# OSU-Bee-Lab/buzzdetect

Measured on AMD Instinct MI355X. Metric: yamnet_windows_per_s, higher is better.
Workload: dtype f32 (split-f16x3 MFMA products, f32 accumulate)

## Files before the change

### buzzdetect_amd/csrc/bd_internal.h

```cpp
#pragma once

#include <hip/hip_runtime.h>
#include <stdint.h>

#include <vector>

#include "../../include/buzzdetect_hip.h"

namespace bd {

constexpr int kMelNonZero = 461;

constexpr int kMelStart[BD_MEL_BANDS] = {
    5, 5, 6, 7, 9, 10, 11, 12, 13, 14, 16, 17, 18, 20, 21, 23, 25, 26, 28, 30, 32, 34, 36, 38, 40, 42, 44, 47, 49, 52, 54, 57,
    60, 63, 66, 69, 72, 76, 79, 83, 87, 90, 95, 99, 103, 108, 112, 117, 122, 127, 133, 138, 144, 150, 156, 162, 169, 176, 183,
    190, 198, 206, 214, 223};
constexpr int kMelLen[BD_MEL_BANDS] = {
    1, 2, 3, 3, 2, 2, 2, 2, 3, 3, 2, 3, 3, 3, 4, 3, 3, 4, 4, 4, 4, 4, 4, 4, 4, 5, 5, 5, 5, 5, 6, 6,
    6, 6, 6, 7, 7, 7, 8, 7, 8, 9, 8, 9, 9, 9, 10, 10, 11, 11, 11, 12, 12, 12, 13, 14, 14, 14, 15, 16, 16, 17, 17, 17};
constexpr int mel_offset(int band) {
    int o = 0;
    for (int m = 0; m < band; ++m) o += kMelLen[m];
    return o;
}
// ... 96 lines not shown
                                   unsigned* range_flag = nullptr);
void launch_scale_copy(const float* src, float* dst, int64_t n, float factor, hipStream_t stream);
bool launch_pointwise_next_dw_f32(const float* in, float* out, int windows, const SepLayer& L, const SepLayer& Ln,
                                  hipStream_t stream);
bool launch_l4_reg_f32(const float* in, float* out, int windows, const SepLayer& L4, const SepLayer& L5, hipStream_t stream);
bool launch_separable_chip(const float* in, float* out, int windows, const SepLayer* L, int nl, hipStream_t stream,
                           const SepLayer* next = nullptr, bool planes = false);
bool tail_supported(const SepLayer& L13, const SepLayer& L14);
bool launch_tail_pw13_dw14(const void* in, void* out, int windows, const SepLayer& L13, const SepLayer& L14, hipStream_t stream);
bool launch_tail_pw14_pool(const void* in, float* pooled, int windows, const SepLayer& L14, hipStream_t stream);
bool tail_f32_supported(const SepLayer& L13, const SepLayer& L14);
bool launch_tail_f32(const float* in, float* mid, float* pooled, int windows, const SepLayer& L13, const SepLayer& L14, hipStream_t stream,
                     int which);
bool launch_separable_chip_f32(const float* in, float* out, int windows, const SepLayer* L, int nl, hipStream_t stream,
                               const SepLayer* next, bool dw0_done);
bool launch_separable_mid_f32(const float* in, float* out, int windows, const SepLayer& L5, const SepLayer& L6, const SepLayer& L7,
                              hipStream_t stream);
bool launch_separable_mid(const float* in, float* out, int windows, const SepLayer& L5, const SepLayer& L6, const SepLayer& L7,
                          hipStream_t stream);
int launch_separable_run_next_dw(const float* a, float* b, int windows, const SepLayer* L, int max_layers, hipStream_t stream,
                                 bool planes = false);
bool launch_separable_fused_next_dw(const float* in, float* out, int windows, const SepLayer& L, const SepLayer& next,
                                    hipStream_t stream);
void launch_stem_reg(const float* logmel, int patch_step, const WindowMap& map, int w0, int windows, const float* c1_w,
                     const float* c1_b, const SepLayer& L2, const SepLayer& L3, float* out, hipStream_t stream);
void launch_stem_reg_f32(const float* logmel, int patch_step, const WindowMap& map, int w0, int windows, const float* c1_w,
                         const float* c1_b, const SepLayer& L2, const SepLayer& L3, float* out, hipStream_t stream);
void launch_stem4(const float* logmel, int patch_step, const WindowMap& map, int w0, int windows, const float* c1_w,
                  const float* c1_b,
                  const SepLayer& L2, const SepLayer& L3, float* out, hipStream_t stream);
void launch_pool_head(const float* act, int windows, const float* head_wt, const float* head_b,
                      int n_classes, float* emb, float* logits, hipStream_t stream);
void launch_head(const float* pooled, int windows, const float* head_wt, const float* head_b, int n_classes,
                 float* logits, hipStream_t stream);

}
```

### buzzdetect_amd/csrc/cnn.hip

```cpp
#include "bd_internal.h"
#include <mutex>
#include <type_traits>

namespace bd {

namespace {

typedef float f32x16 __attribute__((ext_vector_type(16)));

constexpr float kF16Max = 65504.0f;
__device__ __forceinline__ float range_of(float m, float4 v) {
    return fmaxf(fmaxf(m, fabsf(v.x)), fmaxf(fmaxf(fabsf(v.y), fabsf(v.z)), fabsf(v.w)));
}
typedef float v4f_range __attribute__((ext_vector_type(4)));
__device__ __forceinline__ float range_of(float m, v4f_range v) {
    return fmaxf(fmaxf(m, fabsf(v.x)), fmaxf(fmaxf(fabsf(v.y), fabsf(v.z)), fabsf(v.w)));
}
__device__ __forceinline__ void range_report(float m, unsigned* __restrict__ flag) {
    if (flag && !(m <= kF16Max)) *flag = 1u;
}

constexpr int kMaxDevices = 64;
template <typename Kernel>
void allow_dynamic_lds(Kernel kernel, int bytes, std::once_flag (&once)[kMaxDevices]) {
// ... 1207 lines not shown
    }
#undef BD_R_LOAD
#undef BD_R_SPLIT1
    range_report(rmax, range_flag);
}

template <int K16, bool PLAIN = false>
void launch_pw_res(const float* X, const SepLayer& L, float* out, int M, hipStream_t stream) {
    if constexpr (!PLAIN) {
        if (L.pw_mode == 2) return launch_pw_res<K16, true>(X, L, out, M, stream);
    }
    constexpr int lds = 2 * 2 * 32 * 32 * K16;
    static std::once_flag lds_once[kMaxDevices];
    allow_dynamic_lds(&pw_res_kernel<K16, PLAIN>, lds, lds_once);
    const int tiles_n = L.cout / 256;
    const int n_tiles = (M + 31) / 32;
    int streams = 256 / tiles_n;
    if (streams > n_tiles) streams = (n_tiles + 7) / 8 * 8;
    hipLaunchKernelGGL((pw_res_kernel<K16, PLAIN>), dim3((unsigned)(streams * tiles_n)), dim3(512), lds, stream, X,
                       static_cast<const _Float16*>(L.pw_fhi), static_cast<const _Float16*>(L.pw_flo), L.pw_u, L.pw_b, out, M,
                       L.cout, tiles_n, L.range_flag);
}

template <bool PLAIN>
__global__ __launch_bounds__(768) void l4_window_kernel(
    const float* __restrict__ X, const float* __restrict__ dw_w, const float* __restrict__ dw_b,
    const _Float16* __restrict__ Wfhi, const _Float16* __restrict__ Wflo, const float* __restrict__ pw_u,
    const float* __restrict__ pw_b,
    const float* __restrict__ ndw_w, const float* __restrict__ ndw_b, float* __restrict__ out, int windows,
    unsigned* __restrict__ range_flag) {
    constexpr int H = 24, W = 16, C = 128, K16 = 8, STEPS = H / 2;
    constexpr int COL_B = C * 4;
    constexpr int ROW_B = (W + 1) * COL_B;
    constexpr int RING0 = COL_B;
    constexpr int A0 = RING0 + 8 * ROW_B;
    constexpr int A_HALF = 32 * 2 * C, A_BUF = 2 * A_HALF;
    constexpr int T5 = A0 + 2 * A_BUF;
    constexpr int O5 = T5 + C * 12 * 4;
    constexpr int O5_ROW = (W / 2) * C * 4, O5_BUF = 2 * O5_ROW;
    constexpr size_t WIN_IN = (size_t)H * W * C, WIN_OUT = (size_t)STEPS * (W / 2) * C;
    static_assert(A0 % 512 == 0, "fragment addresses are formed by XOR");
    static_assert((2 * STEPS) % 8 == 0 && STEPS % 2 == 0, "ring slots and buffer parities carry over from window to window");
    extern __shared__ __attribute__((aligned(1024))) char smem_raw[];
    char* const smem = smem_raw;
    const int tid = threadIdx.x, lane = tid & 63;
    const int wave = __builtin_amdgcn_readfirstlane(tid >> 6);
    const int b = blockIdx.x, G = gridDim.x;
    if (b >= windows) return;
    const int NT = STEPS * ((windows - b + G - 1) / G);

    for (int i = tid; i < 9 * 32; i += 768) {
        const int z = i >> 5;
        *reinterpret_cast<v4f*>(smem + (z == 0 ? 0 : RING0 + (z - 1) * ROW_B + W * COL_B) + (i & 31) * 16) = v4f{0.f, 0.f, 0.f, 0.f};
    }
    for (int i = tid; i < 10 * C; i += 768) {
        const int t = i / C, c = i - t * C;
        reinterpret_cast<float*>(smem + T5)[c * 12 + t] = t < 9 ? ndw_w[t * C + c] : ndw_b[c];
    }
    float rmax = 0.0f;

    if (wave < 4) {
        const int frow = lane & 31, fh = lane >> 5;
        const int c4 = tid & 31, col_lo = tid >> 5;
        const float* const xt = X + (size_t)b * WIN_IN + (size_t)col_lo * C + c4 * 4;
        char* const ring_t = smem + RING0 + col_lo * COL_B + c4 * 16;
        v4f rs[2][4];
#define BD_L4_LOAD(DST, J)                                                                                \
    {                                                                                                     \
        const int i_ = (J) / STEPS, j_ = (J) - i_ * STEPS;                                                \
        const float* const src_ = xt + (size_t)i_ * G * WIN_IN + (size_t)j_ * (2 * W * C);                \
        _Pragma("unroll") for (int u = 0; u < 4; ++u)                                                     \
            DST[u] = *reinterpret_cast<const v4f*>(src_ + ((u >> 1) * W + 8 * (u & 1)) * C);              \
    }
#define BD_L4_STORE(SRC, J)                                                                               \
    _Pragma("unroll") for (int u = 0; u < 4; ++u)                                                         \
        *reinterpret_cast<v4f*>(ring_t + ((2 * (J) + (u >> 1)) & 7) * ROW_B + 8 * (u & 1) * COL_B) = SRC[u];
        BD_L4_LOAD(rs[0], 0)
        BD_L4_LOAD(rs[1], 1)
        f16x8 bh[K16], bl[K16];
#pragma unroll
        for (int q = 0; q < K16; ++q) {
            const size_t frag = ((size_t)(wave * K16 + q) * 64 + lane) * 8;
            bh[q] = *reinterpret_cast<const f16x8*>(Wfhi + frag);
            if constexpr (!PLAIN) bl[q] = *reinterpret_cast<const f16x8*>(Wflo + frag);
        }
        const int ncol = 32 * wave + frow;
        const float bcol = pw_b[ncol], ucol = pw_u[ncol];
        const float* const t5 = reinterpret_cast<const float*>(smem + T5) + ncol * 12;
        float acc5[4] = {0.0f, 0.0f, 0.0f, 0.0f};
        float* const o5 = reinterpret_cast<float*>(smem + O5) + (2 * fh) * C + ncol;
        int s5 = 0;
        BD_L4_STORE(rs[0], 0)
        BD_L4_STORE(rs[1], 1)
        BD_L4_LOAD(rs[0], 2)
        BD_L4_LOAD(rs[1], 3)
#pragma unroll
        for (int q = 0; q < K16; ++q) {
            bh[q] = pw_landed(bh[q]);
            if constexpr (!PLAIN) bl[q] = pw_landed(bl[q]);
        }
        const unsigned fr0 = pw_lds_addr(smem) + (unsigned)(A0 + frow * 2 * C + ((fh ^ (frow & 15)) << 4));
        __syncthreads();
        auto step = [&](auto pc, int k) {
            constexpr int p = decltype(pc)::value;
            f32x16 acc;
            if (k >= 1 && k <= NT) {
                const unsigned ab = fr0 + (unsigned)((p ^ 1) * A_BUF);
                using S = PwResSchedule<K16, 0, PLAIN ? 1 : 2>;
#pragma unroll
                for (int e = 0; e < 16; ++e) acc[e] = 0.0f;
                f16x8 fa[3][2];
#pragma unroll
                for (int q = 0; q < 2; ++q) {
                    fa[q][0] = pw_lds_frag<0>(ab ^ (q << 5));
                    if constexpr (!PLAIN) fa[q][1] = pw_lds_frag<A_HALF>(ab ^ (q << 5));
                }
                static_for_pw<0, K16>([&](auto qi) {
                    constexpr int q = decltype(qi)::value;
                    if constexpr (q + 2 < K16) {
                        fa[(q + 2) % 3][0] = pw_lds_frag<0>(ab ^ ((q + 2) << 5));
                        if constexpr (!PLAIN) fa[(q + 2) % 3][1] = pw_lds_frag<A_HALF>(ab ^ ((q + 2) << 5));
                    }
                    pw_lds_wait<S::pending(q)>();
                    const f16x8 ah = pw_landed(fa[q % 3][0]);
                    if constexpr (!PLAIN) {
                        const f16x8 al = pw_landed(fa[q % 3][1]);
                        acc = __builtin_amdgcn_mfma_f32_32x32x16_f16(al, bh[q], acc, 0, 0, 0);
                        acc = __builtin_amdgcn_mfma_f32_32x32x16_f16(ah, bl[q], acc, 0, 0, 0);
                    }
                    acc = __builtin_amdgcn_mfma_f32_32x32x16_f16(ah, bh[q], acc, 0, 0, 0);
                });
            }
            if (k + 2 < NT) { BD_L4_STORE(rs[p], k + 2) }
            if (k + 4 < NT) BD_L4_LOAD(rs[p], k + 4)
            if (k >= 1 && k <= NT) {
                float y[2][8], nb[2][2];
                const v4f t5a = *reinterpret_cast<const v4f*>(t5), t5b = *reinterpret_cast<const v4f*>(t5 + 4), t5c = *reinterpret_cast<const v4f*>(t5 + 8);
                const float w5[9] = {t5a.x, t5a.y, t5a.z, t5a.w, t5b.x, t5b.y, t5b.z, t5b.w, t5c.x};
                const float b5 = t5c.y;
#pragma unroll
                for (int e = 0; e < 16; ++e) y[e >> 3][e & 7] = fmaxf(fmaf(acc[e], ucol, bcol), 0.0f);
#pragma unroll
                for (int r = 0; r < 2; ++r) {
                    float va = y[r][0], wa = y[r][4], vb = y[r][4], wb = 0.0f;
                    asm("" : "+v"(va), "+v"(wa), "+v"(vb), "+v"(wb));
                    const auto s1 = __builtin_amdgcn_permlane32_swap(__builtin_bit_cast(unsigned, va), __builtin_bit_cast(unsigned, wa), false, false);
                    const auto s2 = __builtin_amdgcn_permlane32_swap(__builtin_bit_cast(unsigned, vb), __builtin_bit_cast(unsigned, wb), false, false);
                    nb[r][0] = __builtin_bit_cast(float, fh ? (unsigned)s1[0] : (unsigned)s1[1]);
                    nb[r][1] = fh ? 0.0f : __builtin_bit_cast(float, (unsigned)s2[1]);
                }
#define BD_L4_IN(R, T, KW) ((T) == 0 ? y[R][KW] : (T) == 1 ? ((KW) < 2 ? y[R][2 + (KW)] : nb[R][0]) : (T) == 2 ? y[R][4 + (KW)] : ((KW) < 2 ? y[R][6 + (KW)] : nb[R][1]))
                float* const orow = o5 + (p ^ 1) * (O5_BUF / 4);
                if (s5 > 0) {
#pragma unroll
                    for (int t = 0; t < 4; ++t) {
#pragma unroll
                        for (int kw = 0; kw < 3; ++kw) acc5[t] = fmaf(BD_L4_IN(0, t, kw), w5[6 + kw], acc5[t]);
// ... 1 lines not shown
                    }
                }
#pragma unroll
                for (int t = 0; t < 4; ++t) {
                    acc5[t] = b5;
#pragma unroll
                    for (int kh = 0; kh < 2; ++kh)
#pragma unroll
                        for (int kw = 0; kw < 3; ++kw) acc5[t] = fmaf(BD_L4_IN(kh, t, kw), w5[3 * kh + kw], acc5[t]);
                }
                if (s5 == STEPS - 1) {
#pragma unroll
                    for (int t = 0; t < 4; ++t) {
#pragma unroll
                        for (int kw = 0; kw < 3; ++kw) acc5[t] = fmaf(0.0f, w5[6 + kw], acc5[t]);
                        orow[((W / 2) + (t >> 1) * 4 + (t & 1)) * C] = fmaxf(acc5[t], 0.0f);
                    }
                    s5 = 0;
                } else {
                    ++s5;
                }
#undef BD_L4_IN
            }
            __syncthreads();
        };
        for (int k = 0; k < NT + 2; k += 2) {
            step(std::integral_constant<int, 0>{}, k);
            step(std::integral_constant<int, 1>{}, k + 1);
        }
#undef BD_L4_LOAD
#undef BD_L4_STORE
    } else {
        const int v = wave - 4, c4 = lane & 31;
        const int col = v < 4 ? 2 * (2 * v + (lane >> 5)) : 2 * (2 * (v - 4) + (lane >> 5)) + 1;
        v4f w4[9];
#pragma unroll
        for (int t = 0; t < 9; ++t) w4[t] = *reinterpret_cast<const v4f*>(dw_w + t * C + c4 * 4);
        const v4f b4 = *reinterpret_cast<const v4f*>(dw_b + c4 * 4);
        const char* const xin = smem + RING0 + (col - 1) * COL_B + c4 * 16;
        int a_st[2];
#pragma unroll
        for (int rr = 0; rr < 2; ++rr) {
            const int m = 16 * rr + col;
            a_st[rr] = A0 + m * 2 * C + (((c4 >> 1) ^ (m & 15)) << 4) + (c4 & 1) * 8;
        }
        v4f xr[4][3];
        int s4 = 0;
        const int o_lane = (v & 3) * 64 + lane;
        float* const ot = out + (size_t)b * WIN_OUT + (size_t)o_lane * 4;
        int s5 = 0, i5 = 0;
        __syncthreads();
        auto step = [&](auto pc, int k) {
            constexpr int p = decltype(pc)::value;
            if (v < 4 && k >= 2) {
                const char* const ob = smem + O5 + p * O5_BUF + o_lane * 16;
                float* const orow = ot + (size_t)i5 * G * WIN_OUT;
                if (s5 > 0) *reinterpret_cast<v4f*>(orow + (size_t)(s5 - 1) * (W / 2) * C) = *reinterpret_cast<const v4f*>(ob);
                if (s5 == STEPS - 1) {
                    *reinterpret_cast<v4f*>(orow + (size_t)s5 * (W / 2) * C) = *reinterpret_cast<const v4f*>(ob + O5_ROW);
                    s5 = 0;
                    ++i5;
                } else {
                    ++s5;
                }
            }
            if (k < NT) {
                if (s4 == 0) {
#pragma unroll
                    for (int c = 0; c < 3; ++c) {
                        xr[0][c] = v4f{0.f, 0.f, 0.f, 0.f};
                        xr[1][c] = *reinterpret_cast<const v4f*>(xin + c * COL_B);
                    }
                }
// ... 17 lines not shown
                    for (int kh = 0; kh < 3; ++kh)
#pragma unroll
                        for (int kw = 0; kw < 3; ++kw)
                            a4 = __builtin_elementwise_fma(xr[(2 * p + rr + kh) & 3][kw], w4[kh * 3 + kw], a4);
                    a4.x = fmaxf(a4.x, 0.0f); a4.y = fmaxf(a4.y, 0.0f); a4.z = fmaxf(a4.z, 0.0f); a4.w = fmaxf(a4.w, 0.0f);
                    rmax = range_of(rmax, a4);
                    f16x4 hi, lo;
                    split_f16(a4.x, a4.y, a4.z, a4.w, hi, lo);
                    *reinterpret_cast<f16x4*>(smem + a_st[rr] + p * A_BUF) = hi;
                    if constexpr (!PLAIN) *reinterpret_cast<f16x4*>(smem + a_st[rr] + p * A_BUF + A_HALF) = lo;
                }
                s4 = s4 + 1 == STEPS ? 0 : s4 + 1;
            }
            __syncthreads();
        };
        for (int k = 0; k < NT + 2; k += 2) {
            step(std::integral_constant<int, 0>{}, k);
            step(std::integral_constant<int, 1>{}, k + 1);
        }
    }
    range_report(rmax, range_flag);
}

template <bool PLAIN = false>
void launch_l4_window(const float* X, const SepLayer& L, const SepLayer& next, float* out, int windows, hipStream_t stream) {
    if constexpr (!PLAIN) {
        if (L.pw_mode == 2) return launch_l4_window<true>(X, L, next, out, windows, stream);
    }
    constexpr int lds = 512 + 8 * 17 * 512 + 2 * 2 * 32 * 256 + 128 * 12 * 4 + 2 * 2 * 8 * 128 * 4;
    static std::once_flag lds_once[kMaxDevices];
    allow_dynamic_lds(&l4_window_kernel<PLAIN>, lds, lds_once);
    const int grid = windows < 256 ? windows : 256;
    hipLaunchKernelGGL((l4_window_kernel<PLAIN>), dim3((unsigned)grid), dim3(768), lds, stream, X, dw_w_of(L), dw_b_of(L),
                       static_cast<const _Float16*>(L.pw_fhi), static_cast<const _Float16*>(L.pw_flo), L.pw_u, L.pw_b, dw_w_of(next),
                       dw_b_of(next), out, windows, L.range_flag);
}

template <bool PLAIN>
__global__ __launch_bounds__(256, 3) void stem3_kernel(const float* __restrict__ logmel, int patch_step,
                                                    const WindowMap map, int w0,
                                                    const float* __restrict__ c1_w, const float* __restrict__ c1_b,
                                                    const float* __restrict__ dw2_w, const float* __restrict__ dw2_b,
                                                    const _Float16* __restrict__ Whi, const _Float16* __restrict__ Wlo,
                                                    const float* __restrict__ pw_u, const float* __restrict__ pw_b,
                                                    const float* __restrict__ dw3_w,
                                                    const float* __restrict__ dw3_b, float* __restrict__ out,
                                                    const _Float16* __restrict__ W3fhi, const _Float16* __restrict__ W3flo,
                                                    const float* __restrict__ pw3_u, const float* __restrict__ pw3_b,
                                                    unsigned* __restrict__ range_flag) {
    float rmax = 0.0f;
    constexpr int R2 = 5;
    constexpr int C1R = R2 + 2;
    constexpr int LMR = 2 * C1R + 1;
    constexpr int BM = R2 * 32;
    constexpr int PW = 68;
    constexpr int OFF_C1 = 0;
    constexpr int OFF_AH = OFF_C1 + C1R * 34 * 32 * 4;
    constexpr int OFF_AL = OFF_AH + BM * 64;
// ... 458 lines not shown
}

bool launch_pointwise_ws(const float* in, float* out, int64_t rows, const SepLayer& L, hipStream_t stream) {
    if (rows <= 0 || rows >= (1LL << 31) || L.cin < 128 || L.cin % 64 != 0 || L.cout % 256 != 0) return false;
    if (L.pw_variant16 != 10 && (L.cin == 128 || L.cin == 256) && L.cout <= 2048) {
        if (L.cin == 128) launch_pw_res<8>(in, L, out, (int)rows, stream);
        else launch_pw_res<16>(in, L, out, (int)rows, stream);
        return true;
    }
    launch_sep_ws<0, 1>(in, L, out, rows, stream);
    return true;
}

void launch_pointwise(const float* in, float* out, int64_t rows, const SepLayer& L, hipStream_t stream) {
    const bool f16 = L.pw_mode == 1 || L.pw_mode == 2;
    if (f16 && (L.pw_variant16 == 0 || L.pw_variant16 >= 10) && launch_pointwise_ws(in, out, rows, L, stream)) return;
    if (f16)
        launch_pointwise_f16x3_variant(in, L.pw_whi, L.pw_wlo, L.pw_u, L.pw_b, out, rows, L.cout, L.cin, L.pw_variant16,
                                       stream, L.pw_mode == 2, L.range_flag);
    else
        launch_pointwise_variant(in, L.pw_wt, L.pw_b, out, rows, L.cout, L.cin, L.pw_variant, stream);
}

bool launch_separable_fused_next_dw(const float* in, float* out, int windows, const SepLayer& L, const SepLayer& next,
                                    hipStream_t stream) {
    const int P = L.h_out * L.w_out;
    if (L.stride == 1 && next.stride == 2 && windows > 0 && P == 384 && L.w_out == 16 && L.cin == 128 && L.cout == 128 &&
        next.cin == 128) {
        launch_l4_window(in, L, next, out, windows, stream);
        return true;
    }
    if (L.stride != 1 || next.stride != 2 || windows <= 0 || L.cin < 128 || L.cout % 256 != 0) return false;
    if (!((L.h_out == 12 && L.w_out == 8) || (L.h_out == 6 && L.w_out == 4)) || next.cin != L.cout) return false;
    const long long M = (long long)windows * P;
    if (M >= (1LL << 31)) return false;
    launch_sep_ws<1, 0>(in, L, out, M, stream, &next);
    return true;
}

int launch_separable_run_next_dw(const float* a, float* b, int windows, const SepLayer* L, int max_layers, hipStream_t stream,
                                 bool planes) {
    int n = 0;
    while (n < 5 && n + 1 < max_layers) {
        const SepLayer& l = L[n];
        if (l.stride != 1 || l.cin != 512 || l.cout != 512 || l.h_out != 6 || l.w_out != 4 || l.pw_mode != L[0].pw_mode) return 0;
        ++n;
// ... 37 lines not shown
```

### buzzdetect_amd/csrc/engine.hip

```cpp
#include <cmath>
#include <cstdio>
#include <cstdlib>
#include <cstring>
#include <unistd.h>
#include <memory>
#include <string>
#include <type_traits>
#include <utility>
#include <vector>

#include "bd_internal.h"

namespace {

thread_local std::string g_error;

int fail(int code, const std::string& msg) {
    g_error = msg;
    return code;
}

#define BD_HIP(expr)                                                                            \
    do {                                                                                        \
        hipError_t e_ = (expr);                                                                 \
// ... 812 lines not shown
    for (int l = from; l < 13; ++l) {
        if (stop_stage == 2 * l) return BD_OK;
        const bd::SepLayer& L = sep[l];
        if (fuse_next_dw && !dw_done && l + 1 < 13 && (stop_stage < 0 || stop_stage >= 2 * l + 4) &&
            g.launch(3 + 2 * l, [&] { return bd::launch_separable_fused_next_dw(g.a, g.b, g.gw, L, sep[l + 1], g.stream); })) {
            dw_done = true;
            continue;
        }
        if (!dw_done) g.launch(2 + 2 * l, [&] { bd::launch_depthwise(g.a, g.b, g.gw, L, g.stream); });
        if (stop_stage == 2 * l + 1) return BD_OK;
        pointwise(g, l);
        dw_done = false;
    }
    if (stop_stage < 0)
        g.launch(28, [&] {
            bd::launch_pool_head(g.a, g.gw, g.e->head_wt, g.e->head_b, g.e->n_classes, g.emb, g.logits, g.stream);
        });
    return BD_OK;
}

int pass_f16(Group& g) {
    const bd_engine* e = g.e;
    const bd::SepLayer* sep = g.sep;
    if (e->stem != 0) {
        stem(g, e->stem == 3 ? bd::launch_stem_reg : bd::launch_stem4);
    } else {
        conv1(g);
        walk_layers(g, 0, false, 4);
    }
    if (e->separable == 0) return walk_layers(g, 2, false, -1);
    if (!g.launch(7, [&] { return bd::launch_separable_fused_next_dw(g.a, g.b, g.gw, sep[2], sep[3], g.stream); }))
        return walk_layers(g, 2, false, -1);
    if (!(e->separable == 1 &&
          g.launch(13, [&] { return bd::launch_separable_mid(g.b, g.a, g.gw, sep[3], sep[4], sep[5], g.stream); }))) {
        pointwise(g, 3);
        if (!g.launch(11, [&] { return bd::launch_separable_fused_next_dw(g.a, g.b, g.gw, sep[4], sep[5], g.stream); }))
            return walk_layers(g, 4, false, -1);
        pointwise(g, 5);
    }
    const bool planes = bd::tail_supported(sep[11], sep[12]);
    if (!g.launch(23, [&] { return bd::launch_separable_run_next_dw(g.a, g.b, g.gw, &sep[6], 7, g.stream, planes); }))
        return walk_layers(g, 6, false, -1);
    if (!planes) return walk_layers(g, 11, true, -1);
    float* const pooled = g.emb ? g.emb : g.b;
    if (!g.launch(25, [&] { return bd::launch_tail_pw13_dw14(g.b, g.a, g.gw, sep[11], sep[12], g.stream); }) ||
        !g.launch(27, [&] { return bd::launch_tail_pw14_pool(g.a, pooled, g.gw, sep[12], g.stream); }))
        return fail(BD_EHIP, "septail.hip declined the planes of the on-chip run");
    return head(g, pooled);
}

int pass_f32(Group& g) {
    const bd_engine* e = g.e;
    const bd::SepLayer* sep = g.sep;
    stem(g, bd::launch_stem_reg_f32);
    if (e->separable == 0) return walk_layers(g, 2, false, -1);
// ... 508 lines not shown
```

### buzzdetect_amd/csrc/stemreg.hip

```cpp
#include "bd_internal.h"

#include <type_traits>

namespace bd {

namespace {

typedef float f32x16 __attribute__((ext_vector_type(16)));
typedef _Float16 f16x8 __attribute__((ext_vector_type(8)));
typedef _Float16 f16x4 __attribute__((ext_vector_type(4)));
typedef float v4f __attribute__((ext_vector_type(4)));
typedef float v2f __attribute__((ext_vector_type(2)));

constexpr float kF16MaxReg = 65504.0f;

__device__ __forceinline__ int rg_swz64(int row, int slot) { return row * 64 + ((slot ^ ((row >> 2) & 3)) << 4); }
__device__ __forceinline__ float rg_range(float m, v4f v) {
    return fmaxf(fmaxf(m, fabsf(v.x)), fmaxf(fmaxf(fabsf(v.y), fabsf(v.z)), fabsf(v.w)));
}
__device__ __forceinline__ void rg_split(v4f a, f16x4& hi, f16x4& lo) {
    typedef _Float16 f16x2 __attribute__((ext_vector_type(2)));
    const f16x2 h0 = {(_Float16)a.x, (_Float16)a.y}, h1 = {(_Float16)a.z, (_Float16)a.w};
    f16x2 l0, l1;
    asm("v_fma_mixlo_f16 %0, %1, -1.0, %2 op_sel:[0,0,0] op_sel_hi:[1,0,0]" : "=v"(l0) : "v"(h0), "v"(a.x));
    asm("v_fma_mixhi_f16 %0, %1, -1.0, %2 op_sel:[1,0,0] op_sel_hi:[1,0,0]" : "+v"(l0) : "v"(h0), "v"(a.y));
    asm("v_fma_mixlo_f16 %0, %1, -1.0, %2 op_sel:[0,0,0] op_sel_hi:[1,0,0]" : "=v"(l1) : "v"(h1), "v"(a.z));
    asm("v_fma_mixhi_f16 %0, %1, -1.0, %2 op_sel:[1,0,0] op_sel_hi:[1,0,0]" : "+v"(l1) : "v"(h1), "v"(a.w));
    hi[0] = h0[0]; hi[1] = h0[1]; hi[2] = h1[0]; hi[3] = h1[1];
    lo[0] = l0[0]; lo[1] = l0[1]; lo[2] = l1[0]; lo[3] = l1[1];
}

constexpr int OFF_C1 = 0;
constexpr int OFF_AH = 6 * 34 * 32 * 4;
constexpr int OFF_AL = OFF_AH + 128 * 64;
constexpr int OFF_A3H = OFF_AL + 128 * 64;
constexpr int OFF_A3L = OFF_A3H + 2 * 32 * 64;
constexpr int OFF_HALO = OFF_C1 + (2 * 34 + 1) * 32 * 4;
constexpr int OFF_D2W = OFF_A3L + 2 * 32 * 64;
constexpr int OFF_C1W = OFF_D2W + 10 * 32 * 4;
constexpr int kRegLds = OFF_C1W + 10 * 32 * 4;

template <bool PLAIN>
__global__ __launch_bounds__(256, 3) void stem_reg_kernel(const float* __restrict__ logmel, int patch_step, const WindowMap map, int w0,
                                                          const float* __restrict__ c1_w, const float* __restrict__ c1_b,
                                                          const float* __restrict__ dw2_w, const float* __restrict__ dw2_b,
                                                          const _Float16* __restrict__ Whi, const _Float16* __restrict__ Wlo,
                                                          const float* __restrict__ pw_u, const float* __restrict__ pw_b,
                                                          const float* __restrict__ dw3_w, const float* __restrict__ dw3_b,
                                                          float* __restrict__ out, const _Float16* __restrict__ W3fhi,
                                                          const _Float16* __restrict__ W3flo, const float* __restrict__ pw3_u,
                                                          const float* __restrict__ pw3_b, unsigned* __restrict__ range_flag, int windows) {
    __shared__ __attribute__((aligned(16))) char smem[kRegLds];
    float (*s_lm)[68] = reinterpret_cast<float (*)[68]>(smem + OFF_AH);
    float (*s_c1)[34][32] = reinterpret_cast<float (*)[34][32]>(smem + OFF_C1);
    char* const s_ah = smem + OFF_AH;
    char* const s_al = smem + OFF_AL;
    float* const s_halo = reinterpret_cast<float*>(smem + OFF_HALO);
    const float* const s_d2 = reinterpret_cast<const float*>(smem + OFF_D2W);
    const float* const s_c1w = reinterpret_cast<const float*>(smem + OFF_C1W);

    const int tid = threadIdx.x, lane = tid & 63, wave = tid >> 6;
    const int c4 = tid & 7, col = tid >> 3;
    const int g = wave >> 1, wc = wave & 1;
    const int frow = lane & 31, fh = lane >> 5;
    float rmax = 0.0f;

    typedef const __attribute__((address_space(1))) float* gptr;
    typedef const __attribute__((address_space(1))) v4f* gptr4;
    typedef const __attribute__((address_space(1))) f16x8* gptrh;
    gptr pc1w = (gptr)c1_w, pc1b = (gptr)c1_b, pd2w = (gptr)dw2_w, pd2b = (gptr)dw2_b, pu2 = (gptr)pw_u, pb2 = (gptr)pw_b,
         pd3w = (gptr)dw3_w, pd3b = (gptr)dw3_b, pu3 = (gptr)pw3_u, pb3 = (gptr)pw3_b;
    const __attribute__((address_space(1))) _Float16 *pwh = (const __attribute__((address_space(1))) _Float16*)Whi,
// ... 199 lines not shown
            front(std::integral_constant<int, 4>{}, 4 * ob, (t == t_begin || ob == 11) ? 6 : 4);

            v2f x2[8];
#pragma unroll
            for (int k = 0; k < 8; ++k) {
                float e0 = ev[0][k].x, e1 = ev[0][k].y, c0 = carry[k].x, c1 = carry[k].y;
                asm("" : "+v"(e0), "+v"(e1), "+v"(c0), "+v"(c1));
                const auto s0 = __builtin_amdgcn_permlane32_swap(__builtin_bit_cast(unsigned, e0), __builtin_bit_cast(unsigned, c0), false, false);
                const auto s1 = __builtin_amdgcn_permlane32_swap(__builtin_bit_cast(unsigned, e1), __builtin_bit_cast(unsigned, c1), false, false);
                x2[k] = v2f{__builtin_bit_cast(float, fh ? (unsigned)s0[0] : (unsigned)s0[1]),
                            __builtin_bit_cast(float, fh ? (unsigned)s1[0] : (unsigned)s1[1])};
            }
            if (g == 1) {
                float* const hw = s_halo + ((wc * 2 + fh) * 3) * 32 + frow;
                hw[0] = ev[0][0].x;
                hw[32] = ev[1][0].x;
                hw[64] = x2[0].x;
            }
            float d3w[9];
#pragma unroll
            for (int k = 0; k < 9; ++k) d3w[k] = pd3w[k * 64 + wc * 32 + frow];
            const float d3b = pd3b[wc * 32 + frow];
            f16x8 w3h[4], w3l[4];
#pragma unroll
            for (int q = 0; q < 4; ++q) w3h[q] = *(gptrh)(pw3h + ((size_t)(wave * 4 + q) * 64 + lane) * 8);
            __syncthreads();
            band_to_lds(13);
            float hal[3] = {0.0f, 0.0f, 0.0f};
            if (g == 0) {
                const float* const hr = s_halo + ((wc * 2 + fh) * 3) * 32 + frow;
                hal[0] = hr[0];
                hal[1] = hr[32];
                hal[2] = hr[64];
            }
#pragma unroll
            for (int k = 0; k < 4; ++k) {
                v2f a = v2f{d3b, d3b};
#pragma unroll
                for (int kh = 0; kh < 3; ++kh) {
                    const v2f* const row = kh == 0 ? ev[0] : kh == 1 ? ev[1] : x2;
                    v2f shifted;
                    if (k < 3) asm("v_pk_mov_b32 %0, %1, %2 op_sel:[1,0]" : "=v"(shifted) : "v"(row[k]), "v"(row[k < 3 ? k + 1 : 0]));
                    else shifted = v2f{row[k].y, hal[kh]};
                    a = __builtin_elementwise_fma(row[k], v2f{d3w[kh * 3], d3w[kh * 3]}, a);
                    a = __builtin_elementwise_fma(row[4 + k], v2f{d3w[kh * 3 + 1], d3w[kh * 3 + 1]}, a);
                    a = __builtin_elementwise_fma(shifted, v2f{d3w[kh * 3 + 2], d3w[kh * 3 + 2]}, a);
                }
                {
                    const float v0 = fmaxf(a.x, 0.0f), v1 = fmaxf(a.y, 0.0f);
                    unsigned pkh, pkl;
                    asm volatile("v_cvt_pk_f16_f32 %0, %3, %4\n\t"
                                 "v_fma_mixlo_f16 %1, %0, -1.0, %3 op_sel:[0,0,0] op_sel_hi:[1,0,0]\n\t"
                                 "v_fma_mixhi_f16 %1, %0, -1.0, %4 op_sel:[1,0,0] op_sel_hi:[1,0,0]\n\t"
                                 "v_max3_f32 %2, %2, %3, %4"
                                 : "=&v"(pkh), "=&v"(pkl), "+v"(rmax) : "v"(v0), "v"(v1));
                    const int off0 = wc * (32 * 64) + rg_swz64(fh * 16 + 8 * g + 2 * k, frow >> 3) + (frow & 7) * 2;
                    const int off1 = wc * (32 * 64) + rg_swz64(fh * 16 + 8 * g + 2 * k + 1, frow >> 3) + (frow & 7) * 2;
                    *reinterpret_cast<unsigned short*>(smem + OFF_A3H + off0) = (unsigned short)pkh;
                    *reinterpret_cast<unsigned short*>(smem + OFF_A3H + off1) = (unsigned short)(pkh >> 16);
                    *reinterpret_cast<unsigned short*>(smem + OFF_A3L + off0) = (unsigned short)pkl;
                    *reinterpret_cast<unsigned short*>(smem + OFF_A3L + off1) = (unsigned short)(pkl >> 16);
                }
            }
#pragma unroll
            for (int k = 0; k < 8; ++k) carry[k] = ev[0][k];
            if constexpr (!PLAIN) {
#pragma unroll
                for (int q = 0; q < 4; ++q) w3l[q] = *(gptrh)(pw3l + ((size_t)(wave * 4 + q) * 64 + lane) * 8);
            }
            const int n3 = 32 * wave + frow;
            const float b3 = pb3[n3], u3 = pu3[n3];
            __syncthreads();
            f32x16 acc3;
#pragma unroll
            for (int r = 0; r < 16; ++r) acc3[r] = 0.0f;
#pragma unroll
            for (int q = 0; q < 4; ++q) {
                const int off = (q >> 1) * 32 * 64 + rg_swz64(frow, 2 * (q & 1) + fh);
                const f16x8 ah = *reinterpret_cast<const f16x8*>(smem + OFF_A3H + off);
                const f16x8 al = *reinterpret_cast<const f16x8*>(smem + OFF_A3L + off);
                if constexpr (!PLAIN) {
                    acc3 = __builtin_amdgcn_mfma_f32_32x32x16_f16(al, w3h[q], acc3, 0, 0, 0);
                    acc3 = __builtin_amdgcn_mfma_f32_32x32x16_f16(ah, w3l[q], acc3, 0, 0, 0);
                }
                acc3 = __builtin_amdgcn_mfma_f32_32x32x16_f16(ah, w3h[q], acc3, 0, 0, 0);
            }
            float* dst3 = out + (((size_t)win * 24 + 2 * ob) * 16) * 128;
#pragma unroll
            for (int r = 0; r < 16; ++r) {
                const int m = 4 * fh + (r & 3) + 8 * (r >> 2);
                const v2f t2v = __builtin_elementwise_fma(v2f{acc3[r & ~1], acc3[r | 1]}, v2f{u3, u3}, v2f{b3, b3});
                dst3[(size_t)m * 128 + n3] = fmaxf((r & 1) ? t2v.y : t2v.x, 0.0f);
            }
        }
    }
    if (range_flag && !(rmax <= kF16MaxReg)) *range_flag = 1u;
}

}

void launch_stem_reg(const float* logmel, int patch_step, const WindowMap& map, int w0, int windows, const float* c1_w,
                     const float* c1_b, const SepLayer& L2, const SepLayer& L3, float* out, hipStream_t stream) {
    if (windows <= 0) return;
    long long grid = 3ll * cu_count();
    if (grid > 12ll * windows) grid = 12ll * windows;
#define BD_STEM_REG(PLAIN)                                                                                           \
    hipLaunchKernelGGL((stem_reg_kernel<PLAIN>), dim3((unsigned)grid), dim3(256), 0, stream, logmel, patch_step, map, w0, c1_w,    \
                       c1_b, dw_w_of(L2), dw_b_of(L2), static_cast<const _Float16*>(L2.pw_whi),                           \
                       static_cast<const _Float16*>(L2.pw_wlo), L2.pw_u, L2.pw_b, dw_w_of(L3), dw_b_of(L3), out,            \
                       static_cast<const _Float16*>(L3.pw_fhi), static_cast<const _Float16*>(L3.pw_flo), L3.pw_u, L3.pw_b,  \
                       L2.range_flag, windows)
    if (L2.pw_mode == 2) BD_STEM_REG(true);
    else BD_STEM_REG(false);
#undef BD_STEM_REG
}

}
```

Measured before the change: 1.949 million.

## Move layer-3 pointwise from stem kernel into l4 window kernel via f16 planes

The stem kernel can now stop after the layer-3 depthwise and write its split-f16 hi/lo activation planes straight to global memory, instead of running the layer-3 pointwise GEMM and writing a wide f32 tensor. The l4 window kernel gains a PLANES mode that loads these planes, runs the layer-3 pointwise MFMA itself into its LDS ring, and then continues with layer 4. The goal is to halve intermediate HBM traffic between the two kernels and shift the pointwise work to the kernel with spare MFMA capacity. In exchange the l4 kernel uses more LDS and has extra barriers and compute per step, which could reduce its overlap.

```diff
diff --git a/buzzdetect_amd/csrc/bd_internal.h b/buzzdetect_amd/csrc/bd_internal.h
--- a/buzzdetect_amd/csrc/bd_internal.h
+++ b/buzzdetect_amd/csrc/bd_internal.h
@@ -142,8 +142,13 @@
                                  bool planes = false);
 bool launch_separable_fused_next_dw(const float* in, float* out, int windows, const SepLayer& L, const SepLayer& next,
                                     hipStream_t stream);
+bool l4_window_planes_supported(const SepLayer& L3, const SepLayer& L4, const SepLayer& L5);
+bool launch_l4_window_planes(const void* planes, const SepLayer& L3, const SepLayer& L4, const SepLayer& L5, float* out,
+                             int windows, hipStream_t stream);
 void launch_stem_reg(const float* logmel, int patch_step, const WindowMap& map, int w0, int windows, const float* c1_w,
                      const float* c1_b, const SepLayer& L2, const SepLayer& L3, float* out, hipStream_t stream);
+void launch_stem_reg_planes(const float* logmel, int patch_step, const WindowMap& map, int w0, int windows, const float* c1_w,
+                            const float* c1_b, const SepLayer& L2, const SepLayer& L3, float* out, hipStream_t stream);
 void launch_stem_reg_f32(const float* logmel, int patch_step, const WindowMap& map, int w0, int windows, const float* c1_w,
                          const float* c1_b, const SepLayer& L2, const SepLayer& L3, float* out, hipStream_t stream);
 void launch_stem4(const float* logmel, int patch_step, const WindowMap& map, int w0, int windows, const float* c1_w,
diff --git a/buzzdetect_amd/csrc/cnn.hip b/buzzdetect_amd/csrc/cnn.hip
--- a/buzzdetect_amd/csrc/cnn.hip
+++ b/buzzdetect_amd/csrc/cnn.hip
@@ -1253,13 +1253,14 @@
                        L.cout, tiles_n, L.range_flag);
 }
 
-template <bool PLAIN>
+template <bool PLAIN, bool PLANES>
 __global__ __launch_bounds__(768) void l4_window_kernel(
     const float* __restrict__ X, const float* __restrict__ dw_w, const float* __restrict__ dw_b,
     const _Float16* __restrict__ Wfhi, const _Float16* __restrict__ Wflo, const float* __restrict__ pw_u,
     const float* __restrict__ pw_b,
     const float* __restrict__ ndw_w, const float* __restrict__ ndw_b, float* __restrict__ out, int windows,
-    unsigned* __restrict__ range_flag) {
+    unsigned* __restrict__ range_flag, const _Float16* __restrict__ W3fhi, const _Float16* __restrict__ W3flo,
+    const float* __restrict__ pw3_u, const float* __restrict__ pw3_b) {
     constexpr int H = 24, W = 16, C = 128, K16 = 8, STEPS = H / 2;
     constexpr int COL_B = C * 4;
     constexpr int ROW_B = (W + 1) * COL_B;
@@ -1269,6 +1270,9 @@
     constexpr int T5 = A0 + 2 * A_BUF;
     constexpr int O5 = T5 + C * 12 * 4;
     constexpr int O5_ROW = (W / 2) * C * 4, O5_BUF = 2 * O5_ROW;
+    constexpr int PL0 = O5 + 2 * O5_BUF;
+    constexpr int PL_B = 8192, PL_HALF = 4096;
+    constexpr int W3L = PL0 + 2 * PL_B;
     constexpr size_t WIN_IN = (size_t)H * W * C, WIN_OUT = (size_t)STEPS * (W / 2) * C;
     static_assert(A0 % 512 == 0, "fragment addresses are formed by XOR");
     static_assert((2 * STEPS) % 8 == 0 && STEPS % 2 == 0, "ring slots and buffer parities carry over from window to window");
@@ -1306,8 +1310,28 @@
 #define BD_L4_STORE(SRC, J)                                                                               \
     _Pragma("unroll") for (int u = 0; u < 4; ++u)                                                         \
         *reinterpret_cast<v4f*>(ring_t + ((2 * (J) + (u >> 1)) & 7) * ROW_B + 8 * (u & 1) * COL_B) = SRC[u];
-        BD_L4_LOAD(rs[0], 0)
-        BD_L4_LOAD(rs[1], 1)
+        const char* const pt = reinterpret_cast<const char*>(X) + (size_t)b * STEPS * PL_B + tid * 16;
+        v4f rp[2], rq[2];
+#define BD_L4_PLOAD(DST, J)                                                                               \
+    {                                                                                                     \
+        const int i_ = (J) / STEPS, j_ = (J) - i_ * STEPS;                                                \
+        const char* const src_ = pt + ((size_t)i_ * G * STEPS + j_) * PL_B;                               \
+        DST[0] = *reinterpret_cast<const v4f*>(src_);                                                     \
+        if constexpr (!PLAIN) DST[1] = *reinterpret_cast<const v4f*>(src_ + PL_HALF);                     \
+    }
+#define BD_L4_PSTORE(SRC, J)                                                                              \
+    {                                                                                                     \
+        char* const st_ = smem + PL0 + ((J) & 1) * PL_B + tid * 16;                                       \
+        *reinterpret_cast<v4f*>(st_) = SRC[0];                                                            \
+        if constexpr (!PLAIN) *reinterpret_cast<v4f*>(st_ + PL_HALF) = SRC[1];                            \
+    }
+        if constexpr (PLANES) {
+            BD_L4_PLOAD(rp, 0)
+            BD_L4_PLOAD(rq, 1)
+        } else {
+            BD_L4_LOAD(rs[0], 0)
+            BD_L4_LOAD(rs[1], 1)
+        }
         f16x8 bh[K16], bl[K16];
 #pragma unroll
         for (int q = 0; q < K16; ++q) {
@@ -1317,18 +1341,75 @@
         }
         const int ncol = 32 * wave + frow;
         const float bcol = pw_b[ncol], ucol = pw_u[ncol];
+        f16x8 w3h[PLANES ? 4 : 1];
+        char* const w3l = smem + W3L + (wave * 4 * 64 + lane) * 16;
+        float u3 = 0.0f, b3 = 0.0f;
+        if constexpr (PLANES) {
+#pragma unroll
+            for (int q = 0; q < 4; ++q) {
+                const size_t frag = ((size_t)(wave * 4 + q) * 64 + lane) * 8;
+                w3h[q] = *reinterpret_cast<const f16x8*>(W3fhi + frag);
+                if constexpr (!PLAIN) *reinterpret_cast<f16x8*>(w3l + q * 1024) = *reinterpret_cast<const f16x8*>(W3flo + frag);
+            }
+            u3 = pw3_u[ncol];
+            b3 = pw3_b[ncol];
+        }
+        typedef const __attribute__((address_space(3))) f16x8* lptrh;
+        unsigned pl_a[2];
+        pl_a[0] = pw_lds_addr(smem) + (unsigned)(PL0 + frow * 64 + ((fh ^ ((frow >> 2) & 3)) << 4));
+        pl_a[1] = pl_a[0] ^ 32u;
+        asm("" : "+v"(pl_a[0]), "+v"(pl_a[1]));
+        auto pw3 = [&](auto stage_c, int J) {
+            constexpr int stage = decltype(stage_c)::value;
+            f32x16 acc3;
+#pragma unroll
+            for (int r = 0; r < 16; ++r) acc3[r] = 0.0f;
+#pragma unroll
+            for (int q = 0; q < 4; ++q) {
+                const unsigned a = pl_a[q & 1] + (unsigned)(stage * PL_B + (q >> 1) * 2048);
+                const f16x8 ah = *(lptrh)(size_t)a;
+                if constexpr (!PLAIN) {
+                    const f16x8 al = *(lptrh)(size_t)(a + PL_HALF);
+                    acc3 = __builtin_amdgcn_mfma_f32_32x32x16_f16(al, w3h[q], acc3, 0, 0, 0);
+                    acc3 = __builtin_amdgcn_mfma_f32_32x32x16_f16(ah, *reinterpret_cast<const f16x8*>(w3l + q * 1024), acc3, 0, 0, 0);
+                }
+                acc3 = __builtin_amdgcn_mfma_f32_32x32x16_f16(ah, w3h[q], acc3, 0, 0, 0);
+            }
+            char* const rw = smem + RING0 + ncol * 4;
+#pragma unroll
+            for (int r = 0; r < 16; ++r) {
+                const int m = 4 * fh + (r & 3) + 8 * (r >> 2);
+                *reinterpret_cast<float*>(rw + ((2 * J + (m >> 4)) & 7) * ROW_B + (m & 15) * COL_B) = fmaxf(fmaf(acc3[r], u3, b3), 0.0f);
+            }
+        };
         const float* const t5 = reinterpret_cast<const float*>(smem + T5) + ncol * 12;
         float acc5[4] = {0.0f, 0.0f, 0.0f, 0.0f};
         float* const o5 = reinterpret_cast<float*>(smem + O5) + (2 * fh) * C + ncol;
         int s5 = 0;
-        BD_L4_STORE(rs[0], 0)
-        BD_L4_STORE(rs[1], 1)
-        BD_L4_LOAD(rs[0], 2)
-        BD_L4_LOAD(rs[1], 3)
+        if constexpr (PLANES) {
+            BD_L4_PSTORE(rp, 0)
+            BD_L4_PSTORE(rq, 1)
+            BD_L4_PLOAD(rp, 2)
+            BD_L4_PLOAD(rq, 3)
+        } else {
+            BD_L4_STORE(rs[0], 0)
+            BD_L4_STORE(rs[1], 1)
+            BD_L4_LOAD(rs[0], 2)
+            BD_L4_LOAD(rs[1], 3)
+        }
 #pragma unroll
         for (int q = 0; q < K16; ++q) {
             bh[q] = pw_landed(bh[q]);
             if constexpr (!PLAIN) bl[q] = pw_landed(bl[q]);
+        }
+        if constexpr (PLANES) {
+            __syncthreads();
+            pw3(std::integral_constant<int, 0>{}, 0);
+            __syncthreads();
+            BD_L4_PSTORE(rp, 2)
+            rp[0] = rq[0];
+            rp[1] = rq[1];
+            pw3(std::integral_constant<int, 1>{}, 1);
         }
         const unsigned fr0 = pw_lds_addr(smem) + (unsigned)(A0 + frow * 2 * C + ((fh ^ (frow & 15)) << 4));
         __syncthreads();
@@ -1362,8 +1443,13 @@
                     acc = __builtin_amdgcn_mfma_f32_32x32x16_f16(ah, bh[q], acc, 0, 0, 0);
                 });
             }
-            if (k + 2 < NT) { BD_L4_STORE(rs[p], k + 2) }
-            if (k + 4 < NT) BD_L4_LOAD(rs[p], k + 4)
+            if constexpr (PLANES) {
+                if (k + 3 < NT) BD_L4_PSTORE(rp, k + 3)
+                if (k + 4 < NT) BD_L4_PLOAD(rp, k + 4)
+            } else {
+                if (k + 2 < NT) { BD_L4_STORE(rs[p], k + 2) }
+                if (k + 4 < NT) BD_L4_LOAD(rs[p], k + 4)
+            }
             if (k >= 1 && k <= NT) {
                 float y[2][8], nb[2][2];
                 const v4f t5a = *reinterpret_cast<const v4f*>(t5), t5b = *reinterpret_cast<const v4f*>(t5 + 4), t5c = *reinterpret_cast<const v4f*>(t5 + 8);
@@ -1411,6 +1497,9 @@
                 }
 #undef BD_L4_IN
             }
+            if constexpr (PLANES) {
+                if (k + 2 < NT) pw3(pc, k + 2);
+            }
             __syncthreads();
         };
         for (int k = 0; k < NT + 2; k += 2) {
@@ -1419,6 +1508,8 @@
         }
 #undef BD_L4_LOAD
 #undef BD_L4_STORE
+#undef BD_L4_PLOAD
+#undef BD_L4_PSTORE
     } else {
         const int v = wave - 4, c4 = lane & 31;
         const int col = v < 4 ? 2 * (2 * v + (lane >> 5)) : 2 * (2 * (v - 4) + (lane >> 5)) + 1;
@@ -1438,6 +1529,10 @@
         const int o_lane = (v & 3) * 64 + lane;
         float* const ot = out + (size_t)b * WIN_OUT + (size_t)o_lane * 4;
         int s5 = 0, i5 = 0;
+        if constexpr (PLANES) {
+            __syncthreads();
+            __syncthreads();
+        }
         __syncthreads();
         auto step = [&](auto pc, int k) {
             constexpr int p = decltype(pc)::value;
@@ -1501,18 +1596,24 @@
     range_report(rmax, range_flag);
 }
 
-template <bool PLAIN = false>
+template <bool PLAIN, bool PLANES>
+void launch_l4_window_form(const float* X, const SepLayer* L3, const SepLayer& L, const SepLayer& next, float* out, int windows,
+                           hipStream_t stream) {
+    constexpr int lds = 512 + 8 * 17 * 512 + 2 * 2 * 32 * 256 + 128 * 12 * 4 + 2 * 2 * 8 * 128 * 4 + (PLANES ? (PLAIN ? 2 : 4) * 8192 : 0);
+    static std::once_flag lds_once[kMaxDevices];
+    allow_dynamic_lds(&l4_window_kernel<PLAIN, PLANES>, lds, lds_once);
+    const int grid = windows < 256 ? windows : 256;
+    hipLaunchKernelGGL((l4_window_kernel<PLAIN, PLANES>), dim3((unsigned)grid), dim3(768), lds, stream, X, dw_w_of(L), dw_b_of(L),
+                       static_cast<const _Float16*>(L.pw_fhi), static_cast<const _Float16*>(L.pw_flo), L.pw_u, L.pw_b, dw_w_of(next),
+                       dw_b_of(next), out, windows, L.range_flag,
+                       PLANES ? static_cast<const _Float16*>(L3->pw_fhi) : nullptr,
+                       PLANES ? static_cast<const _Float16*>(L3->pw_flo) : nullptr, PLANES ? L3->pw_u : nullptr,
+                       PLANES ? L3->pw_b : nullptr);
+}
+
 void launch_l4_window(const float* X, const SepLayer& L, const SepLayer& next, float* out, int windows, hipStream_t stream) {
-    if constexpr (!PLAIN) {
-        if (L.pw_mode == 2) return launch_l4_window<true>(X, L, next, out, windows, stream);
-    }
-    constexpr int lds = 512 + 8 * 17 * 512 + 2 * 2 * 32 * 256 + 128 * 12 * 4 + 2 * 2 * 8 * 128 * 4;
-    static std::once_flag lds_once[kMaxDevices];
-    allow_dynamic_lds(&l4_window_kernel<PLAIN>, lds, lds_once);
-    const int grid = windows < 256 ? windows : 256;
-    hipLaunchKernelGGL((l4_window_kernel<PLAIN>), dim3((unsigned)grid), dim3(768), lds, stream, X, dw_w_of(L), dw_b_of(L),
-                       static_cast<const _Float16*>(L.pw_fhi), static_cast<const _Float16*>(L.pw_flo), L.pw_u, L.pw_b, dw_w_of(next),
-                       dw_b_of(next), out, windows, L.range_flag);
+    if (L.pw_mode == 2) launch_l4_window_form<true, false>(X, nullptr, L, next, out, windows, stream);
+    else launch_l4_window_form<false, false>(X, nullptr, L, next, out, windows, stream);
 }
 
 template <bool PLAIN>
@@ -2017,6 +2118,21 @@
         launch_pointwise_variant(in, L.pw_wt, L.pw_b, out, rows, L.cout, L.cin, L.pw_variant, stream);
 }
 
+bool l4_window_planes_supported(const SepLayer& L3, const SepLayer& L4, const SepLayer& L5) {
+    return (L3.pw_mode == 1 || L3.pw_mode == 2) && L4.pw_mode == L3.pw_mode && L3.stride == 2 && L3.cin == 64 &&
+           L3.cout == 128 && L3.h_out == 24 && L3.w_out == 16 && L3.pw_fhi && L3.pw_flo && L4.stride == 1 && L4.h_out == 24 &&
+           L4.w_out == 16 && L4.cin == 128 && L4.cout == 128 && L5.stride == 2 && L5.cin == 128;
+}
+
+bool launch_l4_window_planes(const void* planes, const SepLayer& L3, const SepLayer& L4, const SepLayer& L5, float* out,
+                             int windows, hipStream_t stream) {
+    if (windows <= 0 || !l4_window_planes_supported(L3, L4, L5)) return false;
+    const float* const X = static_cast<const float*>(planes);
+    if (L4.pw_mode == 2) launch_l4_window_form<true, true>(X, &L3, L4, L5, out, windows, stream);
+    else launch_l4_window_form<false, true>(X, &L3, L4, L5, out, windows, stream);
+    return true;
+}
+
 bool launch_separable_fused_next_dw(const float* in, float* out, int windows, const SepLayer& L, const SepLayer& next,
                                     hipStream_t stream) {
     const int P = L.h_out * L.w_out;
diff --git a/buzzdetect_amd/csrc/engine.hip b/buzzdetect_amd/csrc/engine.hip
--- a/buzzdetect_amd/csrc/engine.hip
+++ b/buzzdetect_amd/csrc/engine.hip
@@ -858,15 +858,21 @@
 int pass_f16(Group& g) {
     const bd_engine* e = g.e;
     const bd::SepLayer* sep = g.sep;
-    if (e->stem != 0) {
-        stem(g, e->stem == 3 ? bd::launch_stem_reg : bd::launch_stem4);
+    if (e->stem == 3 && e->separable != 0 && bd::l4_window_planes_supported(sep[1], sep[2], sep[3])) {
+        stem(g, bd::launch_stem_reg_planes);
+        if (!g.launch(7, [&] { return bd::launch_l4_window_planes(g.a, sep[1], sep[2], sep[3], g.b, g.gw, g.stream); }))
+            return fail(BD_EHIP, "l4_window_kernel declined the planes of the stem");
     } else {
-        conv1(g);
-        walk_layers(g, 0, false, 4);
-    }
-    if (e->separable == 0) return walk_layers(g, 2, false, -1);
-    if (!g.launch(7, [&] { return bd::launch_separable_fused_next_dw(g.a, g.b, g.gw, sep[2], sep[3], g.stream); }))
-        return walk_layers(g, 2, false, -1);
+        if (e->stem != 0) {
+            stem(g, e->stem == 3 ? bd::launch_stem_reg : bd::launch_stem4);
+        } else {
+            conv1(g);
+            walk_layers(g, 0, false, 4);
+        }
+        if (e->separable == 0) return walk_layers(g, 2, false, -1);
+        if (!g.launch(7, [&] { return bd::launch_separable_fused_next_dw(g.a, g.b, g.gw, sep[2], sep[3], g.stream); }))
+            return walk_layers(g, 2, false, -1);
+    }
     if (!(e->separable == 1 &&
           g.launch(13, [&] { return bd::launch_separable_mid(g.b, g.a, g.gw, sep[3], sep[4], sep[5], g.stream); }))) {
         pointwise(g, 3);
diff --git a/buzzdetect_amd/csrc/stemreg.hip b/buzzdetect_amd/csrc/stemreg.hip
--- a/buzzdetect_amd/csrc/stemreg.hip
+++ b/buzzdetect_amd/csrc/stemreg.hip
@@ -40,14 +40,14 @@
 constexpr int OFF_C1W = OFF_D2W + 10 * 32 * 4;
 constexpr int kRegLds = OFF_C1W + 10 * 32 * 4;
 
-template <bool PLAIN>
+template <bool PLAIN, bool END_DW3>
 __global__ __launch_bounds__(256, 3) void stem_reg_kernel(const float* __restrict__ logmel, int patch_step, const WindowMap map, int w0,
                                                           const float* __restrict__ c1_w, const float* __restrict__ c1_b,
                                                           const float* __restrict__ dw2_w, const float* __restrict__ dw2_b,
                                                           const _Float16* __restrict__ Whi, const _Float16* __restrict__ Wlo,
                                                           const float* __restrict__ pw_u, const float* __restrict__ pw_b,
                                                           const float* __restrict__ dw3_w, const float* __restrict__ dw3_b,
-                                                          float* __restrict__ out, const _Float16* __restrict__ W3fhi,
+                                                          void* __restrict__ out, const _Float16* __restrict__ W3fhi,
                                                           const _Float16* __restrict__ W3flo, const float* __restrict__ pw3_u,
                                                           const float* __restrict__ pw3_b, unsigned* __restrict__ range_flag, int windows) {
     __shared__ __attribute__((aligned(16))) char smem[kRegLds];
@@ -293,8 +293,10 @@
             for (int k = 0; k < 9; ++k) d3w[k] = pd3w[k * 64 + wc * 32 + frow];
             const float d3b = pd3b[wc * 32 + frow];
             f16x8 w3h[4], w3l[4];
-#pragma unroll
-            for (int q = 0; q < 4; ++q) w3h[q] = *(gptrh)(pw3h + ((size_t)(wave * 4 + q) * 64 + lane) * 8);
+            if constexpr (!END_DW3) {
+#pragma unroll
+                for (int q = 0; q < 4; ++q) w3h[q] = *(gptrh)(pw3h + ((size_t)(wave * 4 + q) * 64 + lane) * 8);
+            }
             __syncthreads();
             band_to_lds(13);
             float hal[3] = {0.0f, 0.0f, 0.0f};
@@ -335,33 +337,45 @@
             }
 #pragma unroll
             for (int k = 0; k < 8; ++k) carry[k] = ev[0][k];
-            if constexpr (!PLAIN) {
-#pragma unroll
-                for (int q = 0; q < 4; ++q) w3l[q] = *(gptrh)(pw3l + ((size_t)(wave * 4 + q) * 64 + lane) * 8);
-            }
-            const int n3 = 32 * wave + frow;
-            const float b3 = pb3[n3], u3 = pu3[n3];
-            __syncthreads();
-            f32x16 acc3;
-#pragma unroll
-            for (int r = 0; r < 16; ++r) acc3[r] = 0.0f;
-#pragma unroll
-            for (int q = 0; q < 4; ++q) {
-                const int off = (q >> 1) * 32 * 64 + rg_swz64(frow, 2 * (q & 1) + fh);
-                const f16x8 ah = *reinterpret_cast<const f16x8*>(smem + OFF_A3H + off);
-                const f16x8 al = *reinterpret_cast<const f16x8*>(smem + OFF_A3L + off);
+            if constexpr (END_DW3) {
+                __syncthreads();
+                typedef __attribute__((address_space(1))) char* gchar;
+                const gchar dst = (gchar)out + ((size_t)win * 12 + ob) * 8192 + tid * 16;
+                const v4f ph = *reinterpret_cast<const v4f*>(smem + OFF_A3H + tid * 16);
+                asm volatile("global_store_dwordx4 %0, %1, off\n\ts_nop 2" : : "v"(dst), "v"(ph) : "memory");
                 if constexpr (!PLAIN) {
-                    acc3 = __builtin_amdgcn_mfma_f32_32x32x16_f16(al, w3h[q], acc3, 0, 0, 0);
-                    acc3 = __builtin_amdgcn_mfma_f32_32x32x16_f16(ah, w3l[q], acc3, 0, 0, 0);
-                }
-                acc3 = __builtin_amdgcn_mfma_f32_32x32x16_f16(ah, w3h[q], acc3, 0, 0, 0);
-            }
-            float* dst3 = out + (((size_t)win * 24 + 2 * ob) * 16) * 128;
-#pragma unroll
-            for (int r = 0; r < 16; ++r) {
-                const int m = 4 * fh + (r & 3) + 8 * (r >> 2);
-                const v2f t2v = __builtin_elementwise_fma(v2f{acc3[r & ~1], acc3[r | 1]}, v2f{u3, u3}, v2f{b3, b3});
-                dst3[(size_t)m * 128 + n3] = fmaxf((r & 1) ? t2v.y : t2v.x, 0.0f);
+                    const v4f pl = *reinterpret_cast<const v4f*>(smem + OFF_A3L + tid * 16);
+                    asm volatile("global_store_dwordx4 %0, %1, off\n\ts_nop 2" : : "v"(dst + 4096), "v"(pl) : "memory");
+                }
+            } else {
+                if constexpr (!PLAIN) {
+#pragma unroll
+                    for (int q = 0; q < 4; ++q) w3l[q] = *(gptrh)(pw3l + ((size_t)(wave * 4 + q) * 64 + lane) * 8);
+                }
+                const int n3 = 32 * wave + frow;
+                const float b3 = pb3[n3], u3 = pu3[n3];
+                __syncthreads();
+                f32x16 acc3;
+#pragma unroll
+                for (int r = 0; r < 16; ++r) acc3[r] = 0.0f;
+#pragma unroll
+                for (int q = 0; q < 4; ++q) {
+                    const int off = (q >> 1) * 32 * 64 + rg_swz64(frow, 2 * (q & 1) + fh);
+                    const f16x8 ah = *reinterpret_cast<const f16x8*>(smem + OFF_A3H + off);
+                    const f16x8 al = *reinterpret_cast<const f16x8*>(smem + OFF_A3L + off);
+                    if constexpr (!PLAIN) {
+                        acc3 = __builtin_amdgcn_mfma_f32_32x32x16_f16(al, w3h[q], acc3, 0, 0, 0);
+                        acc3 = __builtin_amdgcn_mfma_f32_32x32x16_f16(ah, w3l[q], acc3, 0, 0, 0);
+                    }
+                    acc3 = __builtin_amdgcn_mfma_f32_32x32x16_f16(ah, w3h[q], acc3, 0, 0, 0);
+                }
+                float* dst3 = static_cast<float*>(out) + (((size_t)win * 24 + 2 * ob) * 16) * 128;
+#pragma unroll
+                for (int r = 0; r < 16; ++r) {
+                    const int m = 4 * fh + (r & 3) + 8 * (r >> 2);
+                    const v2f t2v = __builtin_elementwise_fma(v2f{acc3[r & ~1], acc3[r | 1]}, v2f{u3, u3}, v2f{b3, b3});
+                    dst3[(size_t)m * 128 + n3] = fmaxf((r & 1) ? t2v.y : t2v.x, 0.0f);
+                }
             }
         }
     }
@@ -370,20 +384,36 @@
 
 }
 
-void launch_stem_reg(const float* logmel, int patch_step, const WindowMap& map, int w0, int windows, const float* c1_w,
-                     const float* c1_b, const SepLayer& L2, const SepLayer& L3, float* out, hipStream_t stream) {
+static void launch_stem_reg_form(const float* logmel, int patch_step, const WindowMap& map, int w0, int windows, const float* c1_w,
+                                 const float* c1_b, const SepLayer& L2, const SepLayer& L3, void* out, hipStream_t stream,
+                                 bool planes) {
     if (windows <= 0) return;
     long long grid = 3ll * cu_count();
     if (grid > 12ll * windows) grid = 12ll * windows;
-#define BD_STEM_REG(PLAIN)                                                                                           \
-    hipLaunchKernelGGL((stem_reg_kernel<PLAIN>), dim3((unsigned)grid), dim3(256), 0, stream, logmel, patch_step, map, w0, c1_w,    \
-                       c1_b, dw_w_of(L2), dw_b_of(L2), static_cast<const _Float16*>(L2.pw_whi),                           \
+#define BD_STEM_REG(PLAIN, END_DW3)                                                                                  \
+    hipLaunchKernelGGL((stem_reg_kernel<PLAIN, END_DW3>), dim3((unsigned)grid), dim3(256), 0, stream, logmel, patch_step, map, w0,   \
+                       c1_w, c1_b, dw_w_of(L2), dw_b_of(L2), static_cast<const _Float16*>(L2.pw_whi),                     \
                        static_cast<const _Float16*>(L2.pw_wlo), L2.pw_u, L2.pw_b, dw_w_of(L3), dw_b_of(L3), out,            \
                        static_cast<const _Float16*>(L3.pw_fhi), static_cast<const _Float16*>(L3.pw_flo), L3.pw_u, L3.pw_b,  \
                        L2.range_flag, windows)
-    if (L2.pw_mode == 2) BD_STEM_REG(true);
-    else BD_STEM_REG(false);
+    if (planes) {
+        if (L2.pw_mode == 2) BD_STEM_REG(true, true);
+        else BD_STEM_REG(false, true);
+    } else {
+        if (L2.pw_mode == 2) BD_STEM_REG(true, false);
+        else BD_STEM_REG(false, false);
+    }
 #undef BD_STEM_REG
 }
 
-}
+void launch_stem_reg(const float* logmel, int patch_step, const WindowMap& map, int w0, int windows, const float* c1_w,
+                     const float* c1_b, const SepLayer& L2, const SepLayer& L3, float* out, hipStream_t stream) {
+    launch_stem_reg_form(logmel, patch_step, map, w0, windows, c1_w, c1_b, L2, L3, out, stream, false);
+}
+
+void launch_stem_reg_planes(const float* logmel, int patch_step, const WindowMap& map, int w0, int windows, const float* c1_w,
+                            const float* c1_b, const SepLayer& L2, const SepLayer& L3, float* out, hipStream_t stream) {
+    launch_stem_reg_form(logmel, patch_step, map, w0, windows, c1_w, c1_b, L2, L3, out, stream, true);
+}
+
+}
```

Result: faster. 1.996 million (median of 6 runs) (+2.4%).
